# magicat777/Audio-Analyzer-OMEGA

Measured on NVIDIA B200. Metric: stream-seconds of 48 kHz stereo analysed/sec (multi-res FFT+LUFS+TP), higher is better.
Workload: dtype f32 (FFT, combine, K-weighting in a float32 delta-form state, sample peaks of the true-peak meter; its four transforms per frame pair in f16x2; tensor-core GEMM on (hi, lo) half operands with fp32 accumulators for the few-bin resolutions) + f64 (meter statistics)

## Files before the change

audio-analyzer-omega_b200/csrc/fft_core.cuh:

```cuda
#pragma once
#include <cuda_runtime.h>
#include <stdint.h>

namespace o4 {

__device__ __forceinline__ float2 cmul(float2 a, float2 b) {
    return make_float2(fmaf(a.x, b.x, -a.y * b.y), fmaf(a.x, b.y, a.y * b.x));
}
__device__ __forceinline__ float2 rot_m45(float2 a, float r) {
    return __fmul2_rn(__fadd2_rn(a, make_float2(a.y, -a.x)), make_float2(r, r));
}
__device__ __forceinline__ float2 rot_m135(float2 a, float r) {
    return __fmul2_rn(__fadd2_rn(make_float2(a.y, -a.x), make_float2(-a.x, -a.y)), make_float2(r, r));
}
__device__ __forceinline__ float2 cmul_elem(float2 a, float2 b) { return __fmul2_rn(a, b); }
__device__ __forceinline__ float2 cadd(float2 a, float2 b) { return __fadd2_rn(a, b); }
__device__ __forceinline__ float2 csub(float2 a, float2 b) { return __fadd2_rn(a, make_float2(-b.x, -b.y)); }
__device__ __forceinline__ float2 mul_mi(float2 a) { return make_float2(a.y, -a.x); }

__host__ __device__ __forceinline__ constexpr int padi(int i) { return i + (i >> 4); }

__device__ __forceinline__ void bf4(float2& x0, float2& x1, float2& x2, float2& x3) {
    float2 a = cadd(x0, x2), b = csub(x0, x2), c = cadd(x1, x3), d = mul_mi(csub(x1, x3));
    x0 = cadd(a, c); x1 = cadd(b, d); x2 = csub(a, c); x3 = csub(b, d);
}
__device__ __forceinline__ void bf2(float2& x0, float2& x1) {
    float2 a = cadd(x0, x1), b = csub(x0, x1);
    x0 = a; x1 = b;
}

__device__ __forceinline__ void bf8(float2* v) {
    const float r = 0.70710678118654752440f;
    float2 e0 = v[0], e1 = v[2], e2 = v[4], e3 = v[6];
    float2 o0 = v[1], o1 = v[3], o2 = v[5], o3 = v[7];
    bf4(e0, e1, e2, e3);
    bf4(o0, o1, o2, o3);
    o1 = rot_m45(o1, r);
    o2 = mul_mi(o2);
    o3 = rot_m135(o3, r);
    v[0] = cadd(e0, o0); v[4] = csub(e0, o0);
    v[1] = cadd(e1, o1); v[5] = csub(e1, o1);
    v[2] = cadd(e2, o2); v[6] = csub(e2, o2);
    v[3] = cadd(e3, o3); v[7] = csub(e3, o3);
}

__device__ __forceinline__ void bf16pt(float2* v) {
    const float c1 = 0.92387953251128675613f;
    const float s1 = 0.38268343236508977173f;
    const float r = 0.70710678118654752440f;
#pragma unroll
    for (int a = 0; a < 4; ++a) bf4(v[a], v[a + 4], v[a + 8], v[a + 12]);
    v[1 + 4]  = cmul(v[1 + 4],  make_float2(c1, -s1));
    v[1 + 8]  = rot_m45(v[1 + 8], r);
    v[1 + 12] = cmul(v[1 + 12], make_float2(s1, -c1));
    v[2 + 4]  = rot_m45(v[2 + 4], r);
    v[2 + 8]  = mul_mi(v[2 + 8]);
    v[2 + 12] = rot_m135(v[2 + 12], r);
    v[3 + 4]  = cmul(v[3 + 4],  make_float2(s1, -c1));
    v[3 + 8]  = rot_m135(v[3 + 8], r);
    v[3 + 12] = cmul(v[3 + 12], make_float2(-c1, s1));
#pragma unroll
    for (int c = 0; c < 4; ++c) bf4(v[4 * c], v[4 * c + 1], v[4 * c + 2], v[4 * c + 3]);
#pragma unroll
    for (int c = 0; c < 4; ++c)
#pragma unroll
        for (int d = c + 1; d < 4; ++d) { float2 tmp = v[4 * c + d]; v[4 * c + d] = v[4 * d + c]; v[4 * d + c] = tmp; }
}

struct Tw4 { float2 w1, w2, w4, w8; };

__device__ __forceinline__ void apply_twiddles(float2* v, const Tw4& t) {
    float2 w3 = cmul(t.w1, t.w2);
    float2 w5 = cmul(t.w1, t.w4);
    float2 w6 = cmul(t.w2, t.w4);
    float2 w7 = cmul(w3, t.w4);
    v[1] = cmul(v[1], t.w1);
    v[2] = cmul(v[2], t.w2);
    v[3] = cmul(v[3], w3);
    v[4] = cmul(v[4], t.w4);
    v[5] = cmul(v[5], w5);
    v[6] = cmul(v[6], w6);
    v[7] = cmul(v[7], w7);
    v[8] = cmul(v[8], t.w8);
    v[9] = cmul(v[9], cmul(t.w1, t.w8));
    v[10] = cmul(v[10], cmul(t.w2, t.w8));
    v[11] = cmul(v[11], cmul(w3, t.w8));
    v[12] = cmul(v[12], cmul(t.w4, t.w8));
    v[13] = cmul(v[13], cmul(w5, t.w8));
    v[14] = cmul(v[14], cmul(w6, t.w8));
    v[15] = cmul(v[15], cmul(w7, t.w8));
}

struct Tw15 { float2 w[15]; };

__device__ __forceinline__ void apply_twiddles(float2* v, const Tw15& t) {
#pragma unroll
    for (int k = 1; k < 16; ++k) v[k] = cmul(v[k], t.w[k - 1]);
}

__device__ __forceinline__ void expand_twiddles(const Tw4& t, Tw15& o) {
    const float2 w3 = cmul(t.w1, t.w2), w5 = cmul(t.w1, t.w4), w6 = cmul(t.w2, t.w4), w7 = cmul(w3, t.w4);
    o.w[0] = t.w1; o.w[1] = t.w2; o.w[2] = w3; o.w[3] = t.w4; o.w[4] = w5; o.w[5] = w6; o.w[6] = w7; o.w[7] = t.w8;
    o.w[8] = cmul(t.w1, t.w8); o.w[9] = cmul(t.w2, t.w8); o.w[10] = cmul(w3, t.w8); o.w[11] = cmul(t.w4, t.w8);
    o.w[12] = cmul(w5, t.w8); o.w[13] = cmul(w6, t.w8); o.w[14] = cmul(w7, t.w8);
}

template <int LOG2M>
struct FftShape {
    static constexpr int M = 1 << LOG2M;
    static constexpr int TPF = M / 16;
    static constexpr int NT = (TPF > 256) ? TPF : 256;
    static constexpr int CONC = NT / TPF;
    static constexpr int BUF = M + M / 16;
    static constexpr int NTW = (LOG2M - 1) / 4;
    static constexpr int TAIL = M >> (4 * (LOG2M / 4));
    static constexpr bool LAST16 = (LOG2M % 4 == 0);
    static constexpr bool PINGPONG = (LOG2M <= 13);
    static constexpr int NBUF = PINGPONG ? 2 : 1;
    static_assert(LOG2M >= 8 && LOG2M <= 14, "supported complex sizes: 256 .. 16384");
};

template <int LOG2M>
struct StageTw {
    Tw4 t[FftShape<LOG2M>::NTW > 0 ? FftShape<LOG2M>::NTW : 1];
};

template <int LOG2M>
__device__ __forceinline__ void load_stage_twiddles(StageTw<LOG2M>& st, const float2* __restrict__ twM, int t) {
    using S = FftShape<LOG2M>;
    int s = 1;
#pragma unroll
    for (int i = 0; i < S::NTW; ++i) {
        int e = (t / s) * s;
        st.t[i].w1 = __ldg(twM + e);
        st.t[i].w2 = __ldg(twM + 2 * e);
        st.t[i].w4 = __ldg(twM + 4 * e);
        st.t[i].w8 = __ldg(twM + 8 * e);
        s *= 16;
    }
}

template <int LOG2M, bool KEEP_LAST_IN_REGS>
__device__ __forceinline__ float2* fft_forward(float2* v, float2* buf0, float2* buf1,
                                               const StageTw<LOG2M>& st, int t, bool active) {
    using S = FftShape<LOG2M>;
    constexpr int TPF = S::TPF;
    constexpr int RSTRIDE = TPF + TPF / 16;
    float2* src = buf0;
    float2* dst = buf0;
    int s = 1;
    const int rbase = padi(t);
#pragma unroll
    for (int i = 0; i < S::NTW; ++i) {
        if (i > 0) {
            if (active) {
#pragma unroll
                for (int j = 0; j < 16; ++j) v[j] = src[rbase + j * RSTRIDE];
            }
            if (!S::PINGPONG) __syncthreads();
        }
        dst = (S::PINGPONG && (i & 1)) ? buf1 : buf0;
        if (active) {
            bf16pt(v);
            apply_twiddles(v, st.t[i]);
            int q = t % s, p = t / s;
            if (s == 1) {
                int wb = 17 * t;
#pragma unroll
                for (int k = 0; k < 16; ++k) dst[wb + k] = v[k];
            } else {
                int wb = padi(q + 16 * s * p);
                int ws = s + s / 16;
#pragma unroll
                for (int k = 0; k < 16; ++k) dst[wb + k * ws] = v[k];
            }
        }
        __syncthreads();
        src = dst;
        s *= 16;
    }
    if (S::LAST16) {
        if (active) {
#pragma unroll
            for (int j = 0; j < 16; ++j) v[j] = src[rbase + j * RSTRIDE];
            bf16pt(v);
            if (!KEEP_LAST_IN_REGS) {
#pragma unroll
                for (int k = 0; k < 16; ++k) src[rbase + k * RSTRIDE] = v[k];
            }
        }
    } else {
        constexpr int R3 = S::TAIL;
        constexpr int SS = S::M / R3;
        constexpr int SSP = SS + SS / 16;
        if (active) {
#pragma unroll
            for (int i = 0; i < 16 / R3; ++i) {
                int qb = padi(t + TPF * i);
#pragma unroll
                for (int j = 0; j < R3; ++j) v[i * R3 + j] = src[qb + j * SSP];
                if (R3 == 2) bf2(v[i * 2], v[i * 2 + 1]);
                if (R3 == 4) bf4(v[i * 4], v[i * 4 + 1], v[i * 4 + 2], v[i * 4 + 3]);
                if (R3 == 8) bf8(v + i * 8);
                if (!KEEP_LAST_IN_REGS) {
#pragma unroll
                    for (int j = 0; j < R3; ++j) src[qb + j * SSP] = v[i * R3 + j];
                }
            }
        }
    }
    if (!KEEP_LAST_IN_REGS) __syncthreads();
    return src;
}

template <int NTHREADS>
__device__ __forceinline__ void group_sync(int g) {
    if (NTHREADS <= 32) {
        __syncwarp();
    } else if (NTHREADS < 256) {
        asm volatile("bar.sync %0, %1;" ::"r"(g + 1), "r"(NTHREADS) : "memory");
    } else {
        __syncthreads();
    }
}

template <int LOG2M>
__host__ __device__ __forceinline__ constexpr int zaddr(int idx) {
    constexpr int G2 = (1 << LOG2M) / 256;
    return (idx & ~15) | ((idx & 15) ^ ((((idx >> 4) & (G2 - 1)) * (16 / G2)) & 15));
}

template <int LOG2M>
struct LocalTw { Tw4 s1, s2; };
template <int LOG2M>
struct LocalTwFull { Tw15 s1, s2; };
template <int LOG2M>
__device__ __forceinline__ void expand_local_twiddles(const LocalTw<LOG2M>& a, LocalTwFull<LOG2M>& o) {
    expand_twiddles(a.s1, o.s1);
    expand_twiddles(a.s2, o.s2);
}

template <int LOG2M>
__device__ __forceinline__ void load_local_twiddles(LocalTw<LOG2M>& st, const float2* __restrict__ twM, int t) {
    constexpr int G2 = (1 << LOG2M) / 256;
    st.s1.w1 = __ldg(twM + t);     st.s1.w2 = __ldg(twM + 2 * t);
    st.s1.w4 = __ldg(twM + 4 * t); st.s1.w8 = __ldg(twM + 8 * t);
    const int e = 16 * (t % G2);
    st.s2.w1 = __ldg(twM + e);     st.s2.w2 = __ldg(twM + 2 * e);
    st.s2.w4 = __ldg(twM + 4 * e); st.s2.w8 = __ldg(twM + 8 * e);
}

#ifndef FFT_LAST_STAGE_SHFL
#define FFT_LAST_STAGE_SHFL 1
#endif
template <int LOG2M, bool KEEP_LAST_IN_REGS, typename TW, typename Mid>
__device__ __forceinline__ void fft_forward_local(float2* v, float2* X, float2* Z, const TW& st,
                                                  int t, int g, bool active, Mid&& mid, unsigned zmask = 0xffffffffu) {
    constexpr int M = 1 << LOG2M;
    constexpr int TPF = M / 16;
    constexpr int G2 = M / 256;
    constexpr int S = 17 * G2;
    static_assert(LOG2M >= 8 && LOG2M <= 12, "local variant covers 256 .. 4096 complex points");
    if (active) {
        bf16pt(v);
        apply_twiddles(v, st.s1);
#pragma unroll
        for (int k = 0; k < 16; ++k) X[k * S + t] = v[k];
    }
    group_sync<TPF>(g);
    mid();
    if (active) {
        const int q = t / G2, p = t % G2;
        float2* Xq = X + q * S;
#pragma unroll
        for (int j = 0; j < 16; ++j) v[j] = Xq[p + G2 * j];
        bf16pt(v);
        if (G2 == 1) {
            if (!KEEP_LAST_IN_REGS) {
#pragma unroll
                for (int k = 0; k < 16; ++k) Z[zaddr<LOG2M>(q + 16 * k)] = v[k];
            }
        } else if (G2 == 2 && FFT_LAST_STAGE_SHFL) {
            apply_twiddles(v, st.s2);
            const int zq = zaddr<LOG2M>(q + 16 * p);
            const float sgn = p ? -1.f : 1.f;
#pragma unroll
            for (int i = 0; i < 8; ++i) {
                const float2 keep = p ? v[2 * i + 1] : v[2 * i];
                const float2 send = p ? v[2 * i] : v[2 * i + 1];
                float2 recv;
                recv.x = __shfl_xor_sync(0xffffffffu, send.x, 1);
                recv.y = __shfl_xor_sync(0xffffffffu, send.y, 1);
                v[2 * i] = cadd(keep, recv);
                v[2 * i + 1] = cmul_elem(csub(keep, recv), make_float2(sgn, sgn));
                if (!KEEP_LAST_IN_REGS) {
#pragma unroll
                    for (int pq = 0; pq < 2; ++pq)
                        if (zmask & (1u << pq)) Z[zq + 32 * i + 256 * pq] = v[2 * i + pq];
                }
            }
        } else {
            apply_twiddles(v, st.s2);
            __syncwarp();
#pragma unroll
            for (int k = 0; k < 16; ++k) Xq[17 * p + k] = v[k];
            __syncwarp();
            const int zq = zaddr<LOG2M>(q + 16 * p);
#pragma unroll
            for (int i = 0; i < 16 / G2; ++i) {
                const int k = p + G2 * i;
#pragma unroll
                for (int pp = 0; pp < G2; ++pp) v[i * G2 + pp] = Xq[17 * pp + k];
                if (G2 == 2) bf2(v[i * 2], v[i * 2 + 1]);
                if (G2 == 4) bf4(v[i * 4], v[i * 4 + 1], v[i * 4 + 2], v[i * 4 + 3]);
                if (G2 == 8) bf8(v + i * 8);
                if (G2 == 16) bf16pt(v);
                if (!KEEP_LAST_IN_REGS) {
#pragma unroll
                    for (int pq = 0; pq < G2; ++pq)
                        if (zmask & (1u << pq)) Z[zq + 16 * G2 * i + 256 * pq] = v[i * G2 + pq];
                }
            }
        }
    }
    if (!KEEP_LAST_IN_REGS) group_sync<TPF>(g);
}

__device__ __forceinline__ void rfft_pair(float2 Zk, float2 Zm, float2 w, float2& Xk, float2& Xmk) {
    const float2 hf = make_float2(0.5f, 0.5f);
    float2 E = __fmul2_rn(__fadd2_rn(make_float2(Zm.x, -Zm.y), Zk), hf);
    float2 O = __fmul2_rn(__fadd2_rn(make_float2(Zk.y, -Zk.x), make_float2(Zm.y, Zm.x)), hf);
    float2 T = cmul(w, O);
    Xk = cadd(E, T);
    float2 D = csub(E, T);
    Xmk = make_float2(D.x, -D.y);
}

__device__ __forceinline__ float cabs(float2 a) { return sqrtf(fmaf(a.x, a.x, a.y * a.y)); }
__device__ __forceinline__ float cabs_fast(float2 a) {
    float y;
    asm("sqrt.approx.ftz.f32 %0, %1;" : "=f"(y) : "f"(fmaf(a.x, a.x, a.y * a.y)));
    return y;
}

}
```

audio-analyzer-omega_b200/csrc/multires_kernel.cuh:

```cuda
#pragma once
#include "fft_core.cuh"

namespace o4 {

struct MultiresArgs {
    const float* x;
    long long ch_stride;
    long long frame_stride;
    long long frame_off0;
    int n_ch;
    int n_frames;
    int first_frame;
    int rounds;
    const float* window;
    const float* binw;
    const float2* twM;
    const float2* twN;
    float* mag_out;
    float2* cplx_out;
    float* comb_out;
    int T;
    int n_tb;
    const int* tb_idx;
    const int* tb_lo;
    const float* tb_frac;
    float wnum, wden;
    int need_lo, need_cnt;
};

struct ZPadded { static constexpr bool PADDED = true; __device__ static __forceinline__ int at(int i) { return padi(i); } };
template <int LOG2M>
struct ZSwizzled { static constexpr bool PADDED = false; __device__ static __forceinline__ int at(int i) { return zaddr<LOG2M>(i); } };

template <int LOG2M, typename ZA>
__device__ __forceinline__ void multires_epilogue(const MultiresArgs& a, const float2* Z, float* mags, int t,
                                                  size_t row, bool active, const float2* twn, const float* bw) {
    using S = FftShape<LOG2M>;
    constexpr int M = S::M, TPF = S::TPF;
    const bool all_bins = (a.mag_out != nullptr) || (a.cplx_out != nullptr);
    const int need_hi = a.need_lo + a.need_cnt;
    const int zt0 = ZA::at(t);
    const int zm0 = (t == 0) ? (ZA::PADDED ? M + M / 16 : M) : ZA::at(M - t);
    float* mrow = a.mag_out ? a.mag_out + row * (M + 1) : nullptr;
    float2* crow = a.cplx_out ? a.cplx_out + row * (M + 1) : nullptr;
#pragma unroll
    for (int i = 0; i < 9; ++i) {
        const int u = (i < 8) ? t + i * TPF : M / 2;
        if (i == 8 && t != 0) break;
        const int k = u, km = M - u;
        const bool ink = (k >= a.need_lo && k < need_hi);
        const bool inm = (km >= a.need_lo && km < need_hi);
        if (!(all_bins || ink || inm)) continue;
        float mk = 0.f, mm = 0.f;
        float2 Xk = make_float2(0.f, 0.f), Xm = Xk;
        if (active) {
            const float2 Zk = Z[(i < 8) ? zt0 + i * TPF + (ZA::PADDED ? i * (TPF / 16) : 0) : ZA::at(u)];
            const float2 Zm = Z[(i >= 1 && i < 8) ? zm0 - i * TPF - (ZA::PADDED ? i * (TPF / 16) : 0) : ZA::at((M - u) & (M - 1))];
            const float2 w = twn[u];
            rfft_pair(Zk, Zm, w, Xk, Xm);
            if (all_bins || ink) { mk = cabs_fast(Xk); if (bw) mk *= bw[k]; }
            if (all_bins || inm) { mm = cabs_fast(Xm); if (bw) mm *= bw[km]; }
        }
        if (mrow) { mrow[k] = mk; mrow[km] = mm; }
        if (crow) { crow[k] = Xk; crow[km] = Xm; }
        if (ink) mags[k - a.need_lo] = mk;
        if (inm) mags[km - a.need_lo] = mm;
    }
}

template <int LOG2M, typename ZA>
__device__ __forceinline__ void multires_epilogue_fused(const MultiresArgs& a, const float2* Z, float* mags, int t,
                                                        bool active, const float2* twn, const float* bw) {
    using S = FftShape<LOG2M>;
    constexpr int M = S::M, TPF = S::TPF;
    const int lo = a.need_lo, hi = a.need_lo + a.need_cnt;
    const unsigned cnt = (unsigned)a.need_cnt;
    const int zt0 = ZA::at(t);
    const int zm0 = (t == 0) ? (ZA::PADDED ? M + M / 16 : M) : ZA::at(M - t);
#pragma unroll
    for (int i = 0; i < 8; ++i) {
        const bool anyk = ((i + 1) * TPF > lo) && (i * TPF < hi);
        const bool anym = (M - i * TPF >= lo) && (M - (i + 1) * TPF + 1 < hi);
        if (!(anyk || anym)) continue;
        const int u = t + i * TPF, km = M - u;
        float mk = 0.f, mm = 0.f;
        if (active) {
            const float2 Zk = Z[zt0 + i * TPF + (ZA::PADDED ? i * (TPF / 16) : 0)];
            const float2 Zm = Z[(i >= 1) ? zm0 - i * TPF - (ZA::PADDED ? i * (TPF / 16) : 0) : ZA::at((M - u) & (M - 1))];
            float2 Xk, Xm;
            rfft_pair(Zk, Zm, twn[u], Xk, Xm);
            if (anyk) { mk = cabs_fast(Xk); if (bw) mk *= bw[u]; }
            if (anym) { mm = cabs_fast(Xm); if (bw) mm *= bw[km]; }
        }
        if ((unsigned)(u - lo) < cnt) mags[u - lo] = mk;
        if ((unsigned)(km - lo) < cnt) mags[km - lo] = mm;
    }
    if (t == 0 && (unsigned)(M / 2 - lo) < cnt) {
        float mk = 0.f;
        if (active) {
            const float2 Zh = Z[ZA::at(M / 2)];
            float2 Xk, Xm;
            rfft_pair(Zh, Zh, twn[M / 2], Xk, Xm);
            mk = cabs_fast(Xk);
            if (bw) mk *= bw[M / 2];
        }
        mags[M / 2 - lo] = mk;
    }
}

struct CombTables { const int* idx; const int* lo; const float* frac; };

template <int TPF>
__device__ __forceinline__ void multires_combine(const MultiresArgs& a, const float* mags, int t, size_t row, bool active,
                                                 const CombTables tb) {
    float* orow = a.comb_out + row * a.T;
    const bool unit = (a.wnum == a.wden);
    for (int j = t; j < a.n_tb; j += TPF) {
        const int lo = tb.lo[j];
        float val = 0.f;
        if (active && lo >= 0) {
            const float m0 = mags[lo - a.need_lo];
            const float m1 = mags[lo + 1 - a.need_lo];
            const float vi = fmaf(m1 - m0, tb.frac[j], m0);
            val = unit ? vi : __fdividef(vi * a.wnum, a.wden);
        }
        orow[tb.idx[j]] = val;
    }
}

template <int LOG2M>
__global__ void __launch_bounds__(256, 2)
multires_local_kernel(const __grid_constant__ MultiresArgs a) {
    using S = FftShape<LOG2M>;
    constexpr int M = S::M, TPF = S::TPF, CONC = S::CONC, BUF = S::BUF;
    static_assert(S::NT == 256, "local kernel runs 256-thread CTAs");
    extern __shared__ __align__(16) unsigned char smem_raw[];
    float2* bufs = reinterpret_cast<float2*>(smem_raw);
    float* mags_all = reinterpret_cast<float*>(bufs + (size_t)CONC * (BUF + M));

    const int tid = threadIdx.x;
    const int g = tid / TPF;
    const int t = tid % TPF;
    float2* X = bufs + (size_t)g * (BUF + M);
    float2* Z = X + BUF;
    const int mstride = a.need_cnt > 0 ? a.need_cnt : 1;
    float* mags0 = mags_all + (size_t)g * mstride;
    float* mags1 = mags0 + (size_t)CONC * mstride;
    int* s_tb_idx = reinterpret_cast<int*>(mags_all + (size_t)2 * CONC * mstride);
    int* s_tb_lo = s_tb_idx + a.n_tb;
    float* s_tb_frac = reinterpret_cast<float*>(s_tb_lo + a.n_tb);
    constexpr bool STAGE_TW = (LOG2M <= 10);
    float2* s_twn = reinterpret_cast<float2*>(s_tb_frac + a.n_tb + ((3 * a.n_tb) & 1));
    float* s_bw = reinterpret_cast<float*>(s_twn + (STAGE_TW ? M / 2 + 1 : 0));
    for (int j = threadIdx.x; j < a.n_tb; j += 256) {
        s_tb_idx[j] = __ldg(a.tb_idx + j); s_tb_lo[j] = __ldg(a.tb_lo + j); s_tb_frac[j] = __ldg(a.tb_frac + j);
    }
    if (STAGE_TW) {
        for (int j = threadIdx.x; j <= M / 2; j += 256) s_twn[j] = __ldg(a.twN + j);
        if (a.binw) for (int j = threadIdx.x; j <= M; j += 256) s_bw[j] = __ldg(a.binw + j);
    }
    __syncthreads();
    const CombTables ctb{s_tb_idx, s_tb_lo, s_tb_frac};
    const float2* twn = STAGE_TW ? s_twn : a.twN;
    const float* bw = a.binw ? (STAGE_TW ? s_bw : a.binw) : nullptr;

    const int frames_per_cta = a.rounds * CONC;
    const int tiles_per_ch = (a.n_frames + frames_per_cta - 1) / frames_per_cta;
    const int ch = blockIdx.x / tiles_per_ch;
    const int tile = blockIdx.x % tiles_per_ch;
    const int f0 = tile * frames_per_cta;

    LocalTwFull<LOG2M> st;
    {
        LocalTw<LOG2M> st4;
        load_local_twiddles<LOG2M>(st4, a.twM, t);
        expand_local_twiddles<LOG2M>(st4, st);
    }
    const float2* wptr = reinterpret_cast<const float2*>(a.window) + t;
    unsigned zmask = 0xffffffffu;
    if (a.mag_out == nullptr && a.cplx_out == nullptr && a.need_cnt > 0) {
        zmask = 0u;
        const int lo = a.need_lo, hi = a.need_lo + a.need_cnt - 1;
        const int mlo = M - hi, mhi = M - lo;
        for (int pq = 0; pq < (M / 256 > 0 ? M / 256 : 1); ++pq) {
            const int b0 = 256 * pq, b1 = b0 + 255;
            if ((lo <= b1 && hi >= b0) || (mlo <= b1 && mhi >= b0) || (pq == 0 && mhi >= M)) zmask |= 1u << pq;
        }
    }

    const float* xch = a.x + (long long)ch * a.ch_stride + a.frame_off0;
    float2 v[16];
    {
        const int f = f0 + g;
        if (f < a.n_frames && f >= a.first_frame) {
            const float2* px = reinterpret_cast<const float2*>(xch + (long long)f * a.frame_stride);
#pragma unroll
            for (int j = 0; j < 16; ++j) v[j] = __ldg(px + t + j * TPF);
        }
    }

    for (int r = 0; r < a.rounds; ++r) {
        const int f = f0 + r * CONC + g;
        const bool valid = f < a.n_frames;
        const bool active = valid && f >= a.first_frame;
        if (active && a.window) {
#pragma unroll
            for (int j = 0; j < 16; ++j) v[j] = cmul_elem(v[j], __ldg(wptr + j * TPF));
        }
        fft_forward_local<LOG2M, false>(v, X, Z, st, t, g, active, [&]() {
            if (r > 0 && a.comb_out) {
                const int fp = f - CONC;
                if (fp < a.n_frames)
                    multires_combine<TPF>(a, ((r - 1) & 1) ? mags1 : mags0, t, (size_t)ch * a.n_frames + fp,
                                          fp >= a.first_frame, ctb);
            }
        }, zmask);
        {
            const int fn = f + CONC;
            if (r + 1 < a.rounds && fn < a.n_frames && fn >= a.first_frame) {
                const float2* px = reinterpret_cast<const float2*>(xch + (long long)fn * a.frame_stride);
#pragma unroll
                for (int j = 0; j < 16; ++j) v[j] = __ldg(px + t + j * TPF);
            }
        }
        if (valid) {
            if (a.mag_out == nullptr && a.cplx_out == nullptr)
                multires_epilogue_fused<LOG2M, ZSwizzled<LOG2M>>(a, Z, (r & 1) ? mags1 : mags0, t, active, twn, bw);
            else
                multires_epilogue<LOG2M, ZSwizzled<LOG2M>>(a, Z, (r & 1) ? mags1 : mags0, t, (size_t)ch * a.n_frames + f, active,
                                                           twn, bw);
        }
    }
    if (a.comb_out) {
        group_sync<TPF>(g);
        const int fl = f0 + (a.rounds - 1) * CONC + g;
        if (fl < a.n_frames)
            multires_combine<TPF>(a, ((a.rounds - 1) & 1) ? mags1 : mags0, t, (size_t)ch * a.n_frames + fl,
                                  fl >= a.first_frame, ctb);
    }
}

template <int LOG2M>
inline size_t multires_local_smem_bytes(int need_cnt, int n_tb) {
    using S = FftShape<LOG2M>;
    size_t b = (size_t)S::CONC * (S::BUF + S::M) * sizeof(float2) +
               (size_t)2 * S::CONC * (need_cnt > 0 ? need_cnt : 1) * sizeof(float) + (size_t)(3 * n_tb + 2) * 4;
    if (LOG2M <= 10) b += (size_t)(S::M / 2 + 1) * sizeof(float2) + (size_t)(S::M + 1) * sizeof(float);
    return b + 16;
}

template <int LOG2M>
__global__ void __launch_bounds__(FftShape<LOG2M>::NT, (FftShape<LOG2M>::NT <= 256 ? 2 : 1))
multires_kernel(const __grid_constant__ MultiresArgs a) {
    using S = FftShape<LOG2M>;
    constexpr int TPF = S::TPF, CONC = S::CONC, BUF = S::BUF;
    extern __shared__ __align__(16) unsigned char smem_raw[];
    float2* bufs = reinterpret_cast<float2*>(smem_raw);
    float* mags_all = reinterpret_cast<float*>(bufs + (size_t)CONC * S::NBUF * BUF);

    const int tid = threadIdx.x;
    const int g = tid / TPF;
    const int t = tid % TPF;
    float2* buf0 = bufs + (size_t)g * S::NBUF * BUF;
    float2* buf1 = S::PINGPONG ? buf0 + BUF : buf0;
    float* mags = mags_all + (size_t)g * (a.need_cnt > 0 ? a.need_cnt : 1);

    const int frames_per_cta = a.rounds * CONC;
    const int tiles_per_ch = (a.n_frames + frames_per_cta - 1) / frames_per_cta;
    const int ch = blockIdx.x / tiles_per_ch;
    const int tile = blockIdx.x % tiles_per_ch;
    const int f0 = tile * frames_per_cta;

    float2 win[16];
#pragma unroll
    for (int j = 0; j < 16; ++j)
        win[j] = a.window ? __ldg(reinterpret_cast<const float2*>(a.window) + t + j * TPF) : make_float2(1.f, 1.f);
    StageTw<LOG2M> st;
    load_stage_twiddles<LOG2M>(st, a.twM, t);

    const float* xch = a.x + (long long)ch * a.ch_stride + a.frame_off0;
    float2 v[16];
    {
        const int f = f0 + g;
        if (f < a.n_frames && f >= a.first_frame) {
            const float2* px = reinterpret_cast<const float2*>(xch + (long long)f * a.frame_stride);
#pragma unroll
            for (int j = 0; j < 16; ++j) v[j] = __ldg(px + t + j * TPF);
        }
    }

    for (int r = 0; r < a.rounds; ++r) {
        const int f = f0 + r * CONC + g;
        const bool valid = f < a.n_frames;
        const bool active = valid && f >= a.first_frame;
        if (active) {
#pragma unroll
            for (int j = 0; j < 16; ++j) v[j] = cmul_elem(v[j], win[j]);
        }
        const float2* Z = fft_forward<LOG2M, false>(v, buf0, buf1, st, t, active);
        {
            const int fn = f + CONC;
            if (r + 1 < a.rounds && fn < a.n_frames && fn >= a.first_frame) {
                const float2* px = reinterpret_cast<const float2*>(xch + (long long)fn * a.frame_stride);
#pragma unroll
                for (int j = 0; j < 16; ++j) v[j] = __ldg(px + t + j * TPF);
            }
        }
        const size_t row = (size_t)ch * a.n_frames + (valid ? f : 0);
        if (valid) multires_epilogue<LOG2M, ZPadded>(a, Z, mags, t, row, active, a.twN, a.binw);
        __syncthreads();
        if (valid && a.comb_out) multires_combine<TPF>(a, mags, t, row, active, CombTables{a.tb_idx, a.tb_lo, a.tb_frac});
    }
}

template <int LOG2M>
inline size_t multires_smem_bytes(int need_cnt) {
    using S = FftShape<LOG2M>;
    return (size_t)S::CONC * S::NBUF * S::BUF * sizeof(float2) + (size_t)S::CONC * (need_cnt > 0 ? need_cnt : 1) * sizeof(float);
}

}
```

audio-analyzer-omega_b200/csrc/omega4_cuda.cu:

```cuda
#include "../../include/omega4_cuda.h"

#include <cuda_runtime.h>
#include <math.h>
#include <stdio.h>
#include <stdlib.h>
#include <string.h>

#include <algorithm>
#include <map>
#include <mutex>
#include <set>
#include <string>
#include <vector>

#include "bars_kernel.cuh"
#include "blockdft_kernel.cuh"
#include "blockdft_tc_kernel.cuh"
#include "fft_core.cuh"
#include "kweight_kernel.cuh"
#include "kweight32_kernel.cuh"
#include "loudness_kernel.cuh"
#include "misc_kernels.cuh"
#include "multires_kernel.cuh"
#include "stats_kernel.cuh"
#include "truepeak_kernel.cuh"
#include "truepeak16_kernel.cuh"
#include "waterfall_kernel.cuh"

using namespace o4;

static thread_local std::string g_err;

static int fail(int code, const std::string& msg) {
    g_err = msg;
    return code;
}
#define CK(expr)                                                                                   \
    do {                                                                                           \
        cudaError_t e__ = (expr);                                                                  \
        if (e__ != cudaSuccess) {                                                                  \
            char b__[512];                                                                         \
            snprintf(b__, sizeof b__, "%s failed: %s (%s:%d)", #expr, cudaGetErrorString(e__),     \
                     __FILE__, __LINE__);                                                          \
            return fail(OMEGA4_ERR_CUDA, b__);                                                     \
        }                                                                                          \
    } while (0)

extern "C" const char* omega4_last_error(void) { return g_err.c_str(); }
extern "C" int omega4_abi_version(void) { return OMEGA4_ABI_VERSION; }
extern "C" int omega4_device_count(void) {
    int n = 0;
    if (cudaGetDeviceCount(&n) != cudaSuccess) { cudaGetLastError(); return 0; }
    return n;
}

static int ilog2(int n) { int l = 0; while ((1 << l) < n) ++l; return l; }
static bool is_pow2(int n) { return n > 0 && (n & (n - 1)) == 0; }

struct Twiddles { float2* twM = nullptr; float2* twN = nullptr; float2* tw4W = nullptr; };
static std::mutex g_tw_mu;
static std::map<std::pair<int, int>, Twiddles> g_tw;

static int get_twiddles(int device, int log2m, Twiddles* out) {
    std::lock_guard<std::mutex> lk(g_tw_mu);
    auto key = std::make_pair(device, log2m);
    auto it = g_tw.find(key);
    if (it != g_tw.end()) { *out = it->second; return OMEGA4_OK; }
    const int M = 1 << log2m, N = 2 * M;
    const double two_pi = 6.283185307179586476925287;
    std::vector<float2> a(M), b(M / 2 + 1), c(3 * M + 1);
    for (int e = 0; e < M; ++e) a[e] = make_float2((float)cos(two_pi * e / M), (float)-sin(two_pi * e / M));
    for (int k = 0; k <= M / 2; ++k) b[k] = make_float2((float)cos(two_pi * k / N), (float)-sin(two_pi * k / N));
    for (int j = 0; j <= 3 * M; ++j) c[j] = make_float2((float)cos(two_pi * j / (4.0 * N)), (float)sin(two_pi * j / (4.0 * N)));
    Twiddles t;
    CK(cudaMalloc(&t.twM, a.size() * sizeof(float2)));
    CK(cudaMalloc(&t.twN, b.size() * sizeof(float2)));
    CK(cudaMalloc(&t.tw4W, c.size() * sizeof(float2)));
    CK(cudaMemcpy(t.twM, a.data(), a.size() * sizeof(float2), cudaMemcpyHostToDevice));
    CK(cudaMemcpy(t.twN, b.data(), b.size() * sizeof(float2), cudaMemcpyHostToDevice));
    CK(cudaMemcpy(t.tw4W, c.data(), c.size() * sizeof(float2), cudaMemcpyHostToDevice));
    g_tw[key] = t;
    *out = t;
    return OMEGA4_OK;
}

template <int L>
static int launch_multires_t(const MultiresArgs& a, cudaStream_t s) {
    using S = FftShape<L>;
    const int fpc = a.rounds * S::CONC;
    const long long tiles = (a.n_frames + fpc - 1) / fpc;
    const long long grid = tiles * a.n_ch;
    if (grid <= 0) return OMEGA4_OK;
    if (grid > 2147483647LL) return fail(OMEGA4_ERR_INVALID, "multires grid too large");
    if constexpr (L <= 12) {
        const size_t smem = multires_local_smem_bytes<L>(a.need_cnt, a.n_tb);
        CK(cudaFuncSetAttribute(multires_local_kernel<L>, cudaFuncAttributeMaxDynamicSharedMemorySize, (int)smem));
        multires_local_kernel<L><<<(unsigned)grid, 256, smem, s>>>(a);
    } else {
        const size_t smem = multires_smem_bytes<L>(a.need_cnt);
        CK(cudaFuncSetAttribute(multires_kernel<L>, cudaFuncAttributeMaxDynamicSharedMemorySize, (int)smem));
        multires_kernel<L><<<(unsigned)grid, S::NT, smem, s>>>(a);
    }
    CK(cudaGetLastError());
    return OMEGA4_OK;
}

static int launch_multires(int log2m, const MultiresArgs& a, cudaStream_t s) {
    switch (log2m) {
        case 8: return launch_multires_t<8>(a, s);
        case 9: return launch_multires_t<9>(a, s);
        case 10: return launch_multires_t<10>(a, s);
        case 11: return launch_multires_t<11>(a, s);
        case 12: return launch_multires_t<12>(a, s);
        case 13: return launch_multires_t<13>(a, s);
        case 14: return launch_multires_t<14>(a, s);
    }
    return fail(OMEGA4_ERR_UNSUPPORTED, "fft size must be a power of two in 512 .. 32768");
}

static int default_rounds(int n_frames, int conc) {
    int r = 16;
    while (r > 1 && (long long)r * conc > n_frames) r >>= 1;
    return r;
}

static void fill_truepeak_steps(TruePeakArgs* t) {
    const double two_pi = 6.283185307179586476925287;
    for (int p = 1; p <= 3; ++p) {
        for (int j = 0; j < 16; ++j) {
            const int jj = j < 8 ? j : j - 16;
            t->step[p - 1][j] = make_float2((float)cos(two_pi * p * jj / 64.0), (float)sin(two_pi * p * jj / 64.0));
        }
        t->nyq[p - 1] = (float)cos(two_pi * p / 8.0);
    }
}

static int launch_truepeak(const TruePeakArgs& a, cudaStream_t s) {
    constexpr int L = 11;
    using S = FftShape<L>;
    const size_t smem = truepeak_smem_bytes<L>();
    CK(cudaFuncSetAttribute(truepeak_kernel<L>, cudaFuncAttributeMaxDynamicSharedMemorySize, (int)smem));
    const int ppc = a.rounds * S::CONC;
    const int n_pairs = (a.n_frames + 1) / 2;
    const long long grid = (long long)((n_pairs + ppc - 1) / ppc) * a.n_ch;
    if (grid <= 0) return OMEGA4_OK;
    if (grid > 2147483647LL) return fail(OMEGA4_ERR_INVALID, "truepeak grid too large");
    truepeak_kernel<L><<<(unsigned)grid, S::NT, smem, s>>>(a);
    CK(cudaGetLastError());
    return OMEGA4_OK;
}

static int launch_truepeak16(const TruePeakArgs& a, cudaStream_t s) {
    constexpr int L = 11;
    using S = FftShape<L>;
    const size_t smem = truepeak16_smem_bytes<L>();
    CK(cudaFuncSetAttribute(truepeak16_kernel<L>, cudaFuncAttributeMaxDynamicSharedMemorySize, (int)smem));
    const int ppc = a.rounds * S::CONC;
    const int n_pairs = (a.n_frames + 1) / 2;
    const long long grid = (long long)((n_pairs + ppc - 1) / ppc) * a.n_ch;
    if (grid <= 0) return OMEGA4_OK;
    if (grid > 2147483647LL) return fail(OMEGA4_ERR_INVALID, "truepeak grid too large");
    truepeak16_kernel<L><<<(unsigned)grid, S::NT, smem, s>>>(a);
    CK(cudaGetLastError());
    return OMEGA4_OK;
}

template <bool F64, bool WT>
static int launch_kweight_t(const KweightArgs& a, cudaStream_t s) {
    const size_t smem = kweight_smem_bytes();
    CK(cudaFuncSetAttribute(kweight_kernel<F64, WT>, cudaFuncAttributeMaxDynamicSharedMemorySize, (int)smem));
    const int fpc = a.frames_per_warp * KW_WARPS;
    const long long grid = (long long)((a.n_frames + fpc - 1) / fpc) * a.n_ch;
    if (grid <= 0) return OMEGA4_OK;
    if (grid > 2147483647LL) return fail(OMEGA4_ERR_INVALID, "kweight grid too large");
    kweight_kernel<F64, WT><<<(unsigned)grid, KW_WARPS * 32, smem, s>>>(a);
    CK(cudaGetLastError());
    return OMEGA4_OK;
}

static int launch_kweight(const KweightArgs& a, cudaStream_t s) {
    if (a.x_is_f64) return a.weighted_out ? launch_kweight_t<true, true>(a, s) : launch_kweight_t<true, false>(a, s);
    return a.weighted_out ? launch_kweight_t<false, true>(a, s) : launch_kweight_t<false, false>(a, s);
}

static int launch_kweight32(const Kweight32Args& a, cudaStream_t s) {
    const size_t smem = kweight32_smem_bytes();
    CK(cudaFuncSetAttribute(kweight32_kernel, cudaFuncAttributeMaxDynamicSharedMemorySize, (int)smem));
    const int fpc = a.frames_per_warp * KW32_WARPS;
    const long long grid = (long long)((a.n_frames + fpc - 1) / fpc) * a.n_ch;
    if (grid <= 0) return OMEGA4_OK;
    if (grid > 2147483647LL) return fail(OMEGA4_ERR_INVALID, "kweight grid too large");
    kweight32_kernel<<<(unsigned)grid, KW32_WARPS * 32, smem, s>>>(a);
    CK(cudaGetLastError());
    return OMEGA4_OK;
}

static int launch_stats(const StatsArgs& a, cudaStream_t s) {
    if (a.n_ch <= 0) return OMEGA4_OK;
    if (!a.fresh && a.n_frames == 1 && a.first_frame == 0 && !getenv("OMEGA4_STATS_WALK")) {
        stats_push1_kernel<<<a.n_ch, ST_P1_THREADS, 0, s>>>(a);
    } else if (a.fresh) {
        const size_t smem = stats_smem_bytes<false>();
        CK(cudaFuncSetAttribute(stats_kernel<false>, cudaFuncAttributeMaxDynamicSharedMemorySize, (int)smem));
        stats_kernel<false><<<a.n_ch, ST_THREADS, smem, s>>>(a);
    } else {
        const size_t smem = stats_smem_bytes<true>();
        CK(cudaFuncSetAttribute(stats_kernel<true>, cudaFuncAttributeMaxDynamicSharedMemorySize, (int)smem));
        stats_kernel<true><<<a.n_ch, ST_THREADS, smem, s>>>(a);
    }
    CK(cudaGetLastError());
    return OMEGA4_OK;
}

static int launch_s16_convert(const int16_t* in, long long stream_stride, int il, int n_streams, long long n_frames,
                              float* out, long long out_stride, cudaStream_t s) {
    if (n_streams <= 0 || n_frames <= 0) return OMEGA4_OK;
    if (n_streams > 65535) return fail(OMEGA4_ERR_INVALID, "too many streams for one int16 conversion launch (max 65535)");
    const long long per_stream = n_frames * il;
    dim3 grid((unsigned)((per_stream + 1023) / 1024), (unsigned)n_streams);
    s16_deinterleave_kernel<<<grid, 256, 0, s>>>(in, stream_stride, il, n_frames, out, out_stride);
    CK(cudaGetLastError());
    return OMEGA4_OK;
}

static void mat2_mul(const double* a, const double* b, double* c) {
    double r[4] = {a[0] * b[0] + a[1] * b[2], a[0] * b[1] + a[1] * b[3],
                   a[2] * b[0] + a[3] * b[2], a[2] * b[1] + a[3] * b[3]};
    memcpy(c, r, sizeof r);
}

static void build_biquad(const double* b, const double* a, int order, KwBiquad* q) {
    memset(q, 0, sizeof *q);
    const double a0 = a[0];
    q->b0 = b[0] / a0; q->b1 = b[1] / a0; q->b2 = order >= 2 ? b[2] / a0 : 0.0;
    q->a1 = a[1] / a0; q->a2 = order >= 2 ? a[2] / a0 : 0.0;
    q->pad = 3 * (order + 1);
    if (order >= 2) {
        double zi0, zi1;
        const double m00 = 1.0 + q->a1, m01 = -1.0, m10 = q->a2, m11 = 1.0;
        const double r0 = q->b1 - q->a1 * q->b0, r1 = q->b2 - q->a2 * q->b0;
        const double det = m00 * m11 - m01 * m10;
        zi0 = (r0 * m11 - m01 * r1) / det;
        zi1 = (m00 * r1 - m10 * r0) / det;
        q->yi0 = -zi1 / q->a2;
        q->yi1 = (-zi0 + q->a1 * zi1 / q->a2) / q->a2;
    } else {
        const double zi0 = (q->b1 - q->a1 * q->b0) / (1.0 + q->a1);
        q->yi0 = -zi0 / q->a1;
        q->yi1 = 0.0;
    }
    const double Cm[4] = {-q->a1, -q->a2, 1.0, 0.0};
    double P[4] = {Cm[0], Cm[1], Cm[2], Cm[3]};
    for (int i = 0; i < KW_L; ++i) {
        if (i < KW_SUBMAX) { q->g[i][0] = P[0]; q->g[i][1] = P[1]; }
        if (i + 1 == 16) memcpy(q->c16, P, sizeof P);
        if (i + 1 == 17) memcpy(q->c17, P, sizeof P);
        if (i + 1 < KW_L) mat2_mul(Cm, P, P);
    }
    memcpy(q->phi[0], P, sizeof P);
    for (int j = 1; j < 5; ++j) mat2_mul(q->phi[j - 1], q->phi[j - 1], q->phi[j]);
    auto inv_pow = [&](int k, double* out) {
        if (k == 0) { out[0] = 1; out[1] = 0; out[2] = 0; out[3] = 1; return; }
        if (order >= 2) {
            const double det1 = Cm[0] * Cm[3] - Cm[1] * Cm[2];
            const double Ci[4] = {Cm[3] / det1, -Cm[1] / det1, -Cm[2] / det1, Cm[0] / det1};
            double R[4] = {Ci[0], Ci[1], Ci[2], Ci[3]};
            for (int i = 1; i < k; ++i) mat2_mul(Ci, R, R);
            memcpy(out, R, sizeof R);
        } else {
            out[0] = pow(-q->a1, -(double)k); out[1] = 0; out[2] = 0; out[3] = 0;
        }
    };
    inv_pow(KW_PAD - q->pad, q->cinv_f);
    inv_pow(KW_SLACK + KW_PAD - q->pad, q->cinv_b);
}

struct ResInfo {
    int n = 0, log2m = 0, bins = 0;
    float weight = 1.f;
    float* window = nullptr;
    float* binw = nullptr;
    int n_tb = 0;
    int* tb_idx = nullptr;
    int* tb_lo = nullptr;
    float* tb_frac = nullptr;
    int need_lo = 0, need_cnt = 0;
    Twiddles tw;
};

struct SparseRes {
    int r = 0, nk = 0, nt = 0, B = 0, col0 = 0;
    bool td = false;
    int xoff = 0;
    float2* T = nullptr;
    float* kw = nullptr;
    int* tb_pos = nullptr;
};

struct SparseSet {
    int n = 0;
    SparseRes sp[OMEGA4_MAX_RES];
    int of_res[OMEGA4_MAX_RES];
    int cols = 0, qs = 0;
    float* E = nullptr;
    uint8_t* Eimg = nullptr;
    float e_inv = 1.f;
    int n_halves = 0;
    bool fusable = false;
    int nkx = 0;
    short gB[TC_MAX_GROUPS], gX[TC_MAX_GROUPS], gN[TC_MAX_GROUPS], gS[TC_MAX_GROUPS];
    SparseSet() { for (int i = 0; i < OMEGA4_MAX_RES; ++i) of_res[i] = -1; }
    void release() {
        for (int i = 0; i < OMEGA4_MAX_RES; ++i) { cudaFree(sp[i].T); cudaFree(sp[i].kw); cudaFree(sp[i].tb_pos); }
        cudaFree(E); cudaFree(Eimg);
    }
};

struct DevBuf {
    void* p = nullptr;
    size_t cap = 0;
    int ensure(size_t bytes) {
        if (bytes <= cap) return OMEGA4_OK;
        if (p) cudaFree(p);
        p = nullptr; cap = 0;
        CK(cudaMalloc(&p, bytes));
        cap = bytes;
        return OMEGA4_OK;
    }
    void release() { if (p) cudaFree(p); p = nullptr; cap = 0; }
};

struct omega4_bars {
    int device = 0, T = 0, n_valid = 0, p_lo = 0, normalize_max = 0;
    float p_frac = 0.f, scale = 0.8f;
    int* bands = nullptr; float* gain = nullptr; float* sf = nullptr; float* sfc = nullptr;
    DevBuf h_spec, h_out, h_peak, h_state, state_in;
};

static int bars_launch(omega4_bars* b, cudaStream_t s, const float* spec, int n_ch, int n_hops, float* state, int fresh,
                       float* band_values, float* peak_values, DevBuf* state_copy) {
    BarsArgs a;
    memset(&a, 0, sizeof a);
    a.T = b->T; a.n_ch = n_ch; a.n_hops = n_hops; a.n_valid = b->n_valid; a.bands = b->bands; a.gain = b->gain;
    a.sf = b->sf; a.sfc = b->sfc; a.p_lo = b->p_lo; a.p_frac = b->p_frac; a.scale = b->scale;
    a.normalize_max = b->normalize_max; a.fresh = (fresh || !state) ? 1 : 0;
    a.spec = spec; a.bars_out = band_values; a.peaks_out = peak_values; a.state = state;
    const size_t st_bytes = (size_t)n_ch * (1 + b->n_valid) * sizeof(float);
    const size_t smem = bars_smem_bytes(b->T, b->n_valid);
    if (smem > 200 * 1024) return fail(OMEGA4_ERR_UNSUPPORTED, "spectrum too long for the bars kernel");
    if (b->T > 32 * BARS_MAXV) return fail(OMEGA4_ERR_UNSUPPORTED, "spectrum too long for the bars kernel (max 1024 bins)");
    if (b->T <= 512) CK(cudaFuncSetAttribute(bars_kernel<16>, cudaFuncAttributeMaxDynamicSharedMemorySize, (int)smem));
    else CK(cudaFuncSetAttribute(bars_kernel<32>, cudaFuncAttributeMaxDynamicSharedMemorySize, (int)smem));
    a.seg = n_ch >= 1024 ? 4 * BARS_SEG : BARS_SEG;
    const long long grid = (long long)n_ch * ((n_hops + a.seg - 1) / a.seg);
    if (grid > 2147483647LL) return fail(OMEGA4_ERR_INVALID, "bars grid too large");
    if (a.state && !a.fresh && n_hops > a.seg) {
        int rc = state_copy->ensure(st_bytes); if (rc) return rc;
        CK(cudaMemcpyAsync(state_copy->p, a.state, st_bytes, cudaMemcpyDeviceToDevice, s));
        a.state_in = (const float*)state_copy->p;
    }
    if (b->T <= 512) bars_kernel<16><<<(unsigned)grid, BARS_WARPS * 32, smem, s>>>(a);
    else bars_kernel<32><<<(unsigned)grid, BARS_WARPS * 32, smem, s>>>(a);
    CK(cudaGetLastError());
    return OMEGA4_OK;
}

struct BarsReq {
    omega4_bars* b = nullptr;
    float* band_values = nullptr; float* peak_values = nullptr; float* state = nullptr;
    int fresh = 1;
};

struct KernelTime { char name[32]; cudaEvent_t e0, e1; };

struct SideCtx {
    cudaStream_t side = nullptr;
    cudaEvent_t ev_fork = nullptr, ev_tp = nullptr, ev_join = nullptr;
    int ensure() {
        if (side) return OMEGA4_OK;
        CK(cudaStreamCreateWithFlags(&side, cudaStreamNonBlocking));
        CK(cudaEventCreateWithFlags(&ev_fork, cudaEventDisableTiming));
        CK(cudaEventCreateWithFlags(&ev_tp, cudaEventDisableTiming));
        CK(cudaEventCreateWithFlags(&ev_join, cudaEventDisableTiming));
        return OMEGA4_OK;
    }
    void release() {
        if (side) cudaStreamDestroy(side);
        if (ev_fork) cudaEventDestroy(ev_fork);
        if (ev_tp) cudaEventDestroy(ev_tp);
        if (ev_join) cudaEventDestroy(ev_join);
        side = nullptr; ev_fork = ev_tp = ev_join = nullptr;
    }
};

struct omega4_plan {
    int device = 0;
// ... 1803 lines not shown
```

Baseline: 286,000.

## Add one-warp-per-frame register FFT kernel for N=1024/2048 combine-only path

Adds a warp-level FFT kernel for half-sizes 512 and 1024 (real N 1024/2048). Each warp holds a whole frame in registers, does a 32- or 16-point butterfly, transposes through a padded shared strip with only __syncwarp, then runs a second pass and a shuffle-based real-FFT epilogue. It also adds a 32-point butterfly and selects the new kernel when only combined output is requested. This removes block-wide syncs and shared-memory round trips, at the cost of high register pressure and lower occupancy per SM.

```diff
diff --git a/audio-analyzer-omega_b200/csrc/fft_core.cuh b/audio-analyzer-omega_b200/csrc/fft_core.cuh
--- a/audio-analyzer-omega_b200/csrc/fft_core.cuh
+++ b/audio-analyzer-omega_b200/csrc/fft_core.cuh
@@ -65,6 +65,31 @@
     for (int c = 0; c < 4; ++c)
 #pragma unroll
         for (int d = c + 1; d < 4; ++d) { float2 tmp = v[4 * c + d]; v[4 * c + d] = v[4 * d + c]; v[4 * d + c] = tmp; }
+}
+
+__device__ __forceinline__ void bf32pt(float2* v) {
+    const float r = 0.70710678118654752440f;
+    constexpr float c[9] = {1.f, 0.98078528040323044913f, 0.92387953251128675613f, 0.83146961230254523708f,
+                            0.70710678118654752440f, 0.55557023301960222474f, 0.38268343236508977173f,
+                            0.19509032201612826785f, 0.f};
+#pragma unroll
+    for (int j = 0; j < 16; ++j) {
+        const float2 a = v[j], b = v[j + 16];
+        float2 d = csub(a, b);
+        if (j == 4) d = rot_m45(d, r);
+        else if (j == 8) d = mul_mi(d);
+        else if (j == 12) d = rot_m135(d, r);
+        else if (j != 0) d = cmul(d, make_float2(j <= 8 ? c[j] : -c[16 - j], -(j <= 8 ? c[8 - j] : c[j - 8])));
+        v[j] = cadd(a, b);
+        v[j + 16] = d;
+    }
+    bf16pt(v);
+    bf16pt(v + 16);
+    float2 o[32];
+#pragma unroll
+    for (int k = 0; k < 16; ++k) { o[2 * k] = v[k]; o[2 * k + 1] = v[16 + k]; }
+#pragma unroll
+    for (int k = 0; k < 32; ++k) v[k] = o[k];
 }
 
 struct Tw4 { float2 w1, w2, w4, w8; };
diff --git a/audio-analyzer-omega_b200/csrc/multires_kernel.cuh b/audio-analyzer-omega_b200/csrc/multires_kernel.cuh
--- a/audio-analyzer-omega_b200/csrc/multires_kernel.cuh
+++ b/audio-analyzer-omega_b200/csrc/multires_kernel.cuh
@@ -249,6 +249,196 @@
     return b + 16;
 }
 
+#ifndef XMINB32
+#define XMINB32 3
+#endif
+#ifndef XMINB16
+#define XMINB16 2
+#endif
+#ifndef XPF
+#define XPF 0
+#endif
+template <int LOG2M>
+struct WarpFft {
+    static_assert(LOG2M == 9 || LOG2M == 10, "the one-warp transform covers N = 1024 and 2048");
+    static constexpr int M = 1 << LOG2M;
+    static constexpr int P = M / 32;
+    static constexpr int CONC = FftShape<LOG2M>::CONC;
+    static constexpr int NT = 32 * CONC;
+    static constexpr int STRIP = 32 * (P + 1);
+    static constexpr int MINB = (P == 32) ? XMINB32 : XMINB16;
+    __host__ __device__ static constexpr int slot(int m) { return P == 32 ? m : 2 * (m & 7) + (m >> 3); }
+};
+
+template <int LOG2M>
+__device__ __forceinline__ void multires_epilogue_warp(const MultiresArgs& a, const float2* v, float* mags, int lane,
+                                                       const float2* twn, const float* bw) {
+    using W = WarpFft<LOG2M>;
+    constexpr int M = W::M, P = W::P;
+    const int lo = a.need_lo, hi = a.need_lo + a.need_cnt;
+    const unsigned cnt = (unsigned)a.need_cnt;
+    const int src = (32 - lane) & 31;
+#pragma unroll
+    for (int m = 0; m < P / 2; ++m) {
+        const bool anyk = (32 * m + 32 > lo) && (32 * m < hi);
+        const bool anym = (M - 32 * m >= lo) && (M - 32 * m - 31 < hi);
+        if (!(anyk || anym)) continue;
+        const float2 give = (lane == 0) ? v[W::slot((P - m) & (P - 1))] : v[W::slot(P - 1 - m)];
+        float2 Zm;
+        Zm.x = __shfl_sync(0xffffffffu, give.x, src);
+        Zm.y = __shfl_sync(0xffffffffu, give.y, src);
+        const int u = lane + 32 * m, km = M - u;
+        float2 Xk, Xm;
+        rfft_pair(v[W::slot(m)], Zm, twn[u], Xk, Xm);
+        float mk = 0.f, mm = 0.f;
+        if (anyk) { mk = cabs_fast(Xk); if (bw) mk *= bw[u]; }
+        if (anym) { mm = cabs_fast(Xm); if (bw) mm *= bw[km]; }
+        if ((unsigned)(u - lo) < cnt) mags[u - lo] = mk;
+        if ((unsigned)(km - lo) < cnt) mags[km - lo] = mm;
+    }
+    if (lane == 0 && (unsigned)(M / 2 - lo) < cnt) {
+        const float2 Zh = v[W::slot(P / 2)];
+        float2 Xk, Xm;
+        rfft_pair(Zh, Zh, twn[M / 2], Xk, Xm);
+        float mk = cabs_fast(Xk);
+        if (bw) mk *= bw[M / 2];
+        mags[M / 2 - lo] = mk;
+    }
+}
+
+template <int LOG2M>
+__global__ void __launch_bounds__(WarpFft<LOG2M>::NT, WarpFft<LOG2M>::MINB)
+multires_warp_kernel(const __grid_constant__ MultiresArgs a) {
+    using W = WarpFft<LOG2M>;
+    constexpr int M = W::M, P = W::P, CONC = W::CONC, NT = W::NT;
+    extern __shared__ __align__(16) unsigned char smem_raw[];
+    float2* strips = reinterpret_cast<float2*>(smem_raw);
+    float2* s_twn = strips + (size_t)CONC * W::STRIP;
+    float* s_bw = reinterpret_cast<float*>(s_twn + M / 2 + 1);
+    const int mstride = a.need_cnt > 0 ? a.need_cnt : 1;
+    float* mags_all = s_bw + M + 1;
+    int* s_tb_idx = reinterpret_cast<int*>(mags_all + (size_t)CONC * mstride);
+    int* s_tb_lo = s_tb_idx + a.n_tb;
+    float* s_tb_frac = reinterpret_cast<float*>(s_tb_lo + a.n_tb);
+    for (int j = threadIdx.x; j < a.n_tb; j += NT) {
+        s_tb_idx[j] = __ldg(a.tb_idx + j); s_tb_lo[j] = __ldg(a.tb_lo + j); s_tb_frac[j] = __ldg(a.tb_frac + j);
+    }
+    for (int j = threadIdx.x; j <= M / 2; j += NT) s_twn[j] = __ldg(a.twN + j);
+    if (a.binw) for (int j = threadIdx.x; j <= M; j += NT) s_bw[j] = __ldg(a.binw + j);
+    __syncthreads();
+    const CombTables ctb{s_tb_idx, s_tb_lo, s_tb_frac};
+    const float* bw = a.binw ? s_bw : nullptr;
+
+    const int w = threadIdx.x >> 5;
+    const int lane = threadIdx.x & 31;
+    float2* strip = strips + (size_t)w * W::STRIP;
+    float* mags = mags_all + (size_t)w * mstride;
+
+    const int frames_per_cta = a.rounds * CONC;
+    const int tiles_per_ch = (a.n_frames + frames_per_cta - 1) / frames_per_cta;
+    const int ch = blockIdx.x / tiles_per_ch;
+    const int tile = blockIdx.x % tiles_per_ch;
+    const int f0 = tile * frames_per_cta;
+
+    const int p = lane >> 4;
+    float2 tw1[P - 1];
+#pragma unroll
+    for (int k = 1; k < P; ++k) tw1[k - 1] = __ldg(a.twM + lane * k);
+    float2 tw2[P == 16 ? 15 : 1];
+    if constexpr (P == 16) {
+#pragma unroll
+        for (int k = 1; k < 16; ++k) tw2[k - 1] = __ldg(a.twM + 16 * p * k);
+    }
+    const float2* wptr = reinterpret_cast<const float2*>(a.window) + lane;
+
+    const float* xch = a.x + (long long)ch * a.ch_stride + a.frame_off0;
+    float2 v[P];
+    {
+        const int f = f0 + w;
+        if (f < a.n_frames && f >= a.first_frame) {
+            const float2* px = reinterpret_cast<const float2*>(xch + (long long)f * a.frame_stride);
+#pragma unroll
+            for (int j = 0; j < P; ++j) v[j] = __ldg(px + lane + 32 * j);
+        }
+    }
+
+    for (int r = 0; r < a.rounds; ++r) {
+        const int f = f0 + r * CONC + w;
+        const bool valid = f < a.n_frames;
+        const bool active = valid && f >= a.first_frame;
+#if XPF
+        float2 vn[P];
+        {
+            const int fn = f + CONC;
+            if (r + 1 < a.rounds && fn < a.n_frames && fn >= a.first_frame) {
+                const float2* px = reinterpret_cast<const float2*>(xch + (long long)fn * a.frame_stride);
+#pragma unroll
+                for (int j = 0; j < P; ++j) vn[j] = __ldg(px + lane + 32 * j);
+            }
+        }
+#endif
+        if (active) {
+            if (a.window) {
+#pragma unroll
+                for (int j = 0; j < P; ++j) v[j] = cmul_elem(v[j], __ldg(wptr + 32 * j));
+            }
+            if constexpr (P == 32) bf32pt(v); else bf16pt(v);
+#pragma unroll
+            for (int k = 1; k < P; ++k) v[k] = cmul(v[k], tw1[k - 1]);
+#pragma unroll
+            for (int k = 0; k < P; ++k) strip[(P + 1) * lane + k] = v[k];
+            __syncwarp();
+            if constexpr (P == 32) {
+#pragma unroll
+                for (int t = 0; t < 32; ++t) v[t] = strip[33 * t + lane];
+                bf32pt(v);
+            } else {
+                const float2* col = strip + 17 * p + (lane & 15);
+#pragma unroll
+                for (int t = 0; t < 16; ++t) v[t] = col[34 * t];
+                bf16pt(v);
+#pragma unroll
+                for (int k = 1; k < 16; ++k) v[k] = cmul(v[k], tw2[k - 1]);
+                const float sgn = p ? -1.f : 1.f;
+#pragma unroll
+                for (int i = 0; i < 8; ++i) {
+                    const float2 keep = p ? v[2 * i + 1] : v[2 * i];
+                    const float2 send = p ? v[2 * i] : v[2 * i + 1];
+                    float2 recv;
+                    recv.x = __shfl_xor_sync(0xffffffffu, send.x, 16);
+                    recv.y = __shfl_xor_sync(0xffffffffu, send.y, 16);
+                    v[2 * i] = cadd(keep, recv);
+                    v[2 * i + 1] = cmul_elem(csub(keep, recv), make_float2(sgn, sgn));
+                }
+            }
+            multires_epilogue_warp<LOG2M>(a, v, mags, lane, s_twn, bw);
+        }
+#if XPF
+#pragma unroll
+        for (int j = 0; j < P; ++j) v[j] = vn[j];
+#else
+        {
+            const int fn = f + CONC;
+            if (r + 1 < a.rounds && fn < a.n_frames && fn >= a.first_frame) {
+                const float2* px = reinterpret_cast<const float2*>(xch + (long long)fn * a.frame_stride);
+#pragma unroll
+                for (int j = 0; j < P; ++j) v[j] = __ldg(px + lane + 32 * j);
+            }
+        }
+#endif
+        __syncwarp();
+        if (valid) multires_combine<32>(a, mags, lane, (size_t)ch * a.n_frames + f, active, ctb);
+    }
+}
+
+template <int LOG2M>
+inline size_t multires_warp_smem_bytes(int need_cnt, int n_tb) {
+    using W = WarpFft<LOG2M>;
+    return (size_t)W::CONC * W::STRIP * sizeof(float2) + (size_t)(W::M / 2 + 1) * sizeof(float2) +
+           (size_t)(W::M + 1) * sizeof(float) + (size_t)W::CONC * (need_cnt > 0 ? need_cnt : 1) * sizeof(float) +
+           (size_t)3 * n_tb * 4;
+}
+
 template <int LOG2M>
 __global__ void __launch_bounds__(FftShape<LOG2M>::NT, (FftShape<LOG2M>::NT <= 256 ? 2 : 1))
 multires_kernel(const __grid_constant__ MultiresArgs a) {
diff --git a/audio-analyzer-omega_b200/csrc/omega4_cuda.cu b/audio-analyzer-omega_b200/csrc/omega4_cuda.cu
--- a/audio-analyzer-omega_b200/csrc/omega4_cuda.cu
+++ b/audio-analyzer-omega_b200/csrc/omega4_cuda.cu
@@ -92,6 +92,18 @@
     const long long grid = tiles * a.n_ch;
     if (grid <= 0) return OMEGA4_OK;
     if (grid > 2147483647LL) return fail(OMEGA4_ERR_INVALID, "multires grid too large");
+#ifndef XSEL9
+#define XSEL9 1
+#endif
+    if constexpr ((L == 9 && XSEL9) || L == 10) {
+        if (a.mag_out == nullptr && a.cplx_out == nullptr && a.comb_out != nullptr) {
+            const size_t smem = multires_warp_smem_bytes<L>(a.need_cnt, a.n_tb);
+            CK(cudaFuncSetAttribute(multires_warp_kernel<L>, cudaFuncAttributeMaxDynamicSharedMemorySize, (int)smem));
+            multires_warp_kernel<L><<<(unsigned)grid, WarpFft<L>::NT, smem, s>>>(a);
+            CK(cudaGetLastError());
+            return OMEGA4_OK;
+        }
+    }
     if constexpr (L <= 12) {
         const size_t smem = multires_local_smem_bytes<L>(a.need_cnt, a.n_tb);
         CK(cudaFuncSetAttribute(multires_local_kernel<L>, cudaFuncAttributeMaxDynamicSharedMemorySize, (int)smem));
```

New measurement: 290,700 (median of 6 runs). +1.7%, better.
